# vitoplantamura/OnnxStream

Hardware: NVIDIA H100
Metric: SD1.5 UNet 512x512 bs=1 denoise steps/s (one UNet Model::run per step) (higher is better)
Workload: dtype f16

## Files before the change

### onnxstream_b200/csrc/attention_wgmma.cu

```cuda

#include "common.cuh"
#include "tc_ptx.cuh"
#include <cuda.h>
#include <cstdio>

namespace {

using namespace tcptx;

constexpr int BQ = 128;
constexpr int BKV = 128;
constexpr int KV_STAGES = 4;
constexpr int FA_THREADS = 384;
constexpr int FA_CONSUMERS = 256;
constexpr int FA_PRODUCER_REGS = 40, FA_CONSUMER_REGS = 232;

template <int NCH, int BK, int QKS, int KS = KV_STAGES, int PLANES = 1>
struct FaCfg {
    static_assert(QKS <= 4 * NCH && (BK == 32 || BK == 64 || BK == 128), "tile");
    static constexpr int Q_CHUNK = BQ * 128;
    static constexpr int KV_CHUNK = BK * 128;
    static constexpr int Q_PLANE = NCH * Q_CHUNK;
    static constexpr int KV_PLANE = NCH * KV_CHUNK;
    static constexpr int Q_BYTES = PLANES * Q_PLANE;
    static constexpr int KV_BYTES = PLANES * KV_PLANE;
    static constexpr int BARS = Q_BYTES + KS * 2 * KV_BYTES;
    static constexpr int SMEM = BARS + 1024 + 256;
};

struct FaParams {
    int T, Tk, d;
    int kv_tiles;
    float scale_log2;
    __half* out;
    long long ldo;
};

__device__ __forceinline__ uint8_t* fa_prologue(const CUtensorMap* map_q, const CUtensorMap* map_k, const CUtensorMap* map_v, int bar_off,
                                                uint32_t arrivals, int n0, int n1 = 0)
{
    extern __shared__ uint8_t smem_raw[];
    uint8_t* smem = (uint8_t*)(((uintptr_t)smem_raw + 1023) & ~(uintptr_t)1023);
    const int warp = threadIdx.x >> 5, lane = threadIdx.x & 31;
    if (warp == 0 && lane == 0) {
        asm volatile("prefetch.tensormap [%0];" ::"l"(map_q) : "memory");
        asm volatile("prefetch.tensormap [%0];" ::"l"(map_k) : "memory");
        asm volatile("prefetch.tensormap [%0];" ::"l"(map_v) : "memory");
    }
    if (warp == 1 && lane == 0) {
        uint64_t* bars = (uint64_t*)(smem + bar_off);
        mbar_init(bars, 1);
        for (int i = 0; i < n0; i++) { mbar_init(&bars[1 + i], 1); mbar_init(&bars[1 + n0 + i], arrivals); }
        for (int i = 0; i < n1; i++) { mbar_init(&bars[1 + 2 * n0 + i], 1); mbar_init(&bars[1 + 2 * n0 + n1 + i], arrivals); }
        asm volatile("fence.mbarrier_init.release.cluster;" ::: "memory");
    }
    __syncthreads();
    osb_pdl_wait();
    return smem;
}

template <int KS, typename Load>
__device__ __forceinline__ void fa_produce_kv(uint64_t* kv_full, uint64_t* kv_empty, int n_kv, uint32_t tile_bytes, Load load)
{
    for (int j = 0; j < n_kv; j++) {
        const int st = j % KS;
        mbar_wait(&kv_empty[st], ((j / KS) & 1) ^ 1);
        if (elect_one()) {
            mbar_expect_tx(&kv_full[st], tile_bytes);
            load(st, j, &kv_full[st]);
        }
        __syncwarp();
    }
    osb_pdl_trigger_late();
}

template <int BK>
__device__ __forceinline__ float fa_row_max(const float (&s)[BK / 2], int h)
{
    float mt = -INFINITY;
#pragma unroll
    for (int c = 0; c < BK / 8; c++) mt = fmaxf(mt, fmaxf(s[4 * c + 2 * h], s[4 * c + 2 * h + 1]));
    mt = fmaxf(mt, __shfl_xor_sync(0xffffffffu, mt, 1));
    mt = fmaxf(mt, __shfl_xor_sync(0xffffffffu, mt, 2));
    return mt;
}

__device__ __forceinline__ float ex2_approx(float x)
{
    float y;
    asm("ex2.approx.ftz.f32 %0, %1;" : "=f"(y) : "f"(x));
    return y;
}

__device__ __forceinline__ uint32_t pack_half2(float lo, float hi)
{
    __half2 h2 = __floats2half2_rn(lo, hi);
    return *reinterpret_cast<uint32_t*>(&h2);
}

__device__ __forceinline__ void store_pair(__half* p, float lo, float hi) { *reinterpret_cast<uint32_t*>(p) = pack_half2(lo, hi); }
__device__ __forceinline__ void store_pair(float* p, float lo, float hi) { *reinterpret_cast<float2*>(p) = make_float2(lo, hi); }

template <typename OutT, int NCH>
__device__ __forceinline__ void fa_store(const float (&o)[NCH][32], const float (&l_run)[2], OutT* const (&rows)[2], int ncols, int cq)
{
#pragma unroll
    for (int h = 0; h < 2; h++) {
        float l = l_run[h];
        l += __shfl_xor_sync(0xffffffffu, l, 1);
        l += __shfl_xor_sync(0xffffffffu, l, 2);
        const float inv = 1.f / l;
        if (!rows[h]) continue;
#pragma unroll
        for (int ch = 0; ch < NCH; ch++)
#pragma unroll
            for (int c = 0; c < 8; c++) {
                const int col = 64 * ch + 8 * c + cq;
                if (col < ncols) store_pair(rows[h] + col, o[ch][4 * c + 2 * h] * inv, o[ch][4 * c + 2 * h + 1] * inv);
            }
    }
}

template <int BK>
__device__ __forceinline__ void qk_mma(float (&s)[BK / 2], uint64_t da, uint64_t db, uint32_t scale_d = 1u)
{
    if constexpr (BK == 128) wgmma_m64n128k16_f16<0>(s, da, db, scale_d);
    else if constexpr (BK == 64) wgmma_m64n64k16_f16<0>(s, da, db, scale_d);
    else wgmma_m64n32k16_f16<0>(s, da, db, scale_d);
}

template <int NCH, int BK, int QKS>
__device__ __forceinline__ void fa_issue_qk(float (&s)[BK / 2], uint64_t qdesc, uint64_t kdesc)
{
    using C = FaCfg<NCH, BK, QKS>;
    fence_regs(s);
    wgmma_fence();
#pragma unroll
    for (int k = 0; k < QKS; k++)
        qk_mma<BK>(s, qdesc + (uint64_t)(((k >> 2) * C::Q_CHUNK >> 4) + (k & 3) * 2), kdesc + (uint64_t)(((k >> 2) * C::KV_CHUNK >> 4) + (k & 3) * 2), k > 0);
    wgmma_commit();
}

template <int NCH, int BK, int QKS>
__device__ __forceinline__ void fa_issue_pv(float (&o)[NCH][32], uint32_t (&a)[BK / 16][4], uint64_t vdesc)
{
    using C = FaCfg<NCH, BK, QKS>;
#pragma unroll
    for (int ch = 0; ch < NCH; ch++) fence_regs(o[ch]);
    fence_regs(a);
    wgmma_fence();
#pragma unroll
    for (int kk = 0; kk < BK / 16; kk++)
#pragma unroll
        for (int ch = 0; ch < NCH; ch++)
            wgmma_m64n64k16_f16_rs(o[ch], a[kk], vdesc + (uint64_t)((ch * C::KV_CHUNK + kk * 2048) >> 4), 1u);
    wgmma_commit();
}

template <int BK>
__device__ __forceinline__ void fa_softmax(float (&s)[BK / 2], float (&m_run)[2], float (&l_run)[2], float (&alpha)[2], int key0, int cq, const FaParams& p)
{
    if (key0 + BK > p.Tk) {
#pragma unroll
        for (int c = 0; c < BK / 8; c++)
#pragma unroll
            for (int e = 0; e < 2; e++)
                if (key0 + 8 * c + cq + e >= p.Tk) { s[4 * c + e] = -INFINITY; s[4 * c + 2 + e] = -INFINITY; }
    }
    float neg_m[2];
#pragma unroll
    for (int h = 0; h < 2; h++) {
        const float m_new = fmaxf(m_run[h], fa_row_max<BK>(s, h) * p.scale_log2);
        alpha[h] = ex2_approx(m_run[h] - m_new);
        neg_m[h] = -m_new;
        m_run[h] = m_new;
    }
    float lsum[2] = { 0.f, 0.f };
#pragma unroll
    for (int c = 0; c < BK / 8; c++)
#pragma unroll
        for (int h = 0; h < 2; h++)
#pragma unroll
            for (int e = 0; e < 2; e++) {
                const float pe = ex2_approx(fmaf(s[4 * c + 2 * h + e], p.scale_log2, neg_m[h]));
                s[4 * c + 2 * h + e] = pe;
                lsum[h] += pe;
            }
#pragma unroll
    for (int h = 0; h < 2; h++) l_run[h] = l_run[h] * alpha[h] + lsum[h];
}

template <int NCH, int BK>
__device__ __forceinline__ void fa_rescale_pack(float (&o)[NCH][32], uint32_t (&a)[BK / 16][4], const float (&s)[BK / 2], const float (&alpha)[2])
{
#pragma unroll
    for (int ch = 0; ch < NCH; ch++)
#pragma unroll
        for (int c = 0; c < 8; c++)
#pragma unroll
            for (int h = 0; h < 2; h++) { o[ch][4 * c + 2 * h] *= alpha[h]; o[ch][4 * c + 2 * h + 1] *= alpha[h]; }
#pragma unroll
    for (int c = 0; c < BK / 8; c++)
#pragma unroll
        for (int h = 0; h < 2; h++) a[c >> 1][(c & 1) * 2 + h] = pack_half2(s[4 * c + 2 * h], s[4 * c + 2 * h + 1]);
}

template <int NCH, int BK, int QKS>
__global__ void __launch_bounds__(FA_THREADS, 1)
flash_attention_kernel(const __grid_constant__ CUtensorMap map_q, const __grid_constant__ CUtensorMap map_k, const __grid_constant__ CUtensorMap map_v,
                       const FaParams p)
{
    using C = FaCfg<NCH, BK, QKS>;
    constexpr int S = KV_STAGES;
    osb_pdl_trigger_entry();
    const int warp = threadIdx.x >> 5, lane = threadIdx.x & 31;
    const int head = blockIdx.y;
    const int q0 = blockIdx.x * BQ;
    const int n_kv = p.kv_tiles;
    uint8_t* smem = fa_prologue(&map_q, &map_k, &map_v, C::BARS, FA_CONSUMERS / 32, S);
    uint8_t* sQ = smem;
    uint8_t* sK = sQ + C::Q_BYTES;
    uint8_t* sV = sK + S * C::KV_BYTES;
    uint64_t* q_full = (uint64_t*)(smem + C::BARS);
    uint64_t* kv_full = q_full + 1;
    uint64_t* kv_empty = kv_full + S;

    if (warp < 4) {
        setmaxnreg_dec<FA_PRODUCER_REGS>();
        if (warp == 0) {
            if (elect_one()) {
                mbar_expect_tx(q_full, C::Q_BYTES);
#pragma unroll
                for (int c = 0; c < NCH; c++) tma_load_3d(sQ + c * C::Q_CHUNK, &map_q, q_full, 64 * c, head, q0);
            }
            __syncwarp();
            fa_produce_kv<S>(kv_full, kv_empty, n_kv, 2 * C::KV_BYTES, [&](int st, int j, uint64_t* bar) {
#pragma unroll
                for (int c = 0; c < NCH; c++) {
                    tma_load_3d(sK + st * C::KV_BYTES + c * C::KV_CHUNK, &map_k, bar, 64 * c, head, j * BK);
                    tma_load_3d(sV + st * C::KV_BYTES + c * C::KV_CHUNK, &map_v, bar, 64 * c, head, j * BK);
                }
            });
        }
    } else {
        setmaxnreg_inc<FA_CONSUMER_REGS>();
        const int wg = (warp >> 2) - 1;
        const int r = (warp & 3) * 16 + (lane >> 2);
        const int cq = 2 * (lane & 3);
        const uint32_t my_bar = 1 + wg, other_bar = 2 - wg;
        if (wg == 0) named_bar_arrive(my_bar, FA_CONSUMERS);
        const uint64_t qdesc = make_smem_desc(smem_u32(sQ) + wg * (BQ / 2) * 128, 16, 1024);
        const uint64_t kdesc0 = make_smem_desc(smem_u32(sK), 16, 1024);
        const uint64_t vdesc0 = make_smem_desc(smem_u32(sV), C::KV_CHUNK, 1024);
        float o[NCH][32];
#pragma unroll
        for (int ch = 0; ch < NCH; ch++)
#pragma unroll
            for (int i = 0; i < 32; i++) o[ch][i] = 0.f;
        float s[BK / 2];
        uint32_t a[BK / 16][4];
        float m_run[2] = { -INFINITY, -INFINITY }, l_run[2] = { 0.f, 0.f }, alpha[2];
        mbar_wait(q_full, 0);

        mbar_wait(&kv_full[0], 0);
        named_bar_sync(my_bar, FA_CONSUMERS);
        fa_issue_qk<NCH, BK, QKS>(s, qdesc, kdesc0);
        named_bar_arrive(other_bar, FA_CONSUMERS);
        wgmma_wait<0>();
        fence_regs(s);
        fa_softmax<BK>(s, m_run, l_run, alpha, 0, cq, p);
        fa_rescale_pack<NCH, BK>(o, a, s, alpha);
        for (int j = 1; j < n_kv; j++) {
            const int st = j % S, prev = (j - 1) % S;
            mbar_wait(&kv_full[st], (j / S) & 1);
            named_bar_sync(my_bar, FA_CONSUMERS);
            fa_issue_qk<NCH, BK, QKS>(s, qdesc, kdesc0 + (uint64_t)(st * C::KV_BYTES >> 4));
            fa_issue_pv<NCH, BK, QKS>(o, a, vdesc0 + (uint64_t)(prev * C::KV_BYTES >> 4));
            named_bar_arrive(other_bar, FA_CONSUMERS);
            wgmma_wait<1>();
            fence_regs(s);
            fa_softmax<BK>(s, m_run, l_run, alpha, j * BK, cq, p);
            wgmma_wait<0>();
#pragma unroll
            for (int ch = 0; ch < NCH; ch++) fence_regs(o[ch]);
            fence_regs(a);
            __syncwarp();
            if (lane == 0) mbar_arrive(&kv_empty[prev]);
            fa_rescale_pack<NCH, BK>(o, a, s, alpha);
        }
        named_bar_sync(my_bar, FA_CONSUMERS);
        fa_issue_pv<NCH, BK, QKS>(o, a, vdesc0 + (uint64_t)((n_kv - 1) % S * C::KV_BYTES >> 4));
        if (wg == 0) named_bar_arrive(other_bar, FA_CONSUMERS);
        wgmma_wait<0>();
#pragma unroll
        for (int ch = 0; ch < NCH; ch++) fence_regs(o[ch]);
        __half* rows[2];
#pragma unroll
        for (int h = 0; h < 2; h++) {
            const int qrow = q0 + wg * (BQ / 2) + r + 8 * h;
            rows[h] = qrow < p.T ? p.out + (long long)qrow * p.ldo + (long long)head * p.d : nullptr;
        }
        fa_store(o, l_run, rows, p.d, cq);
    }
}

template <auto Kernel, typename... Args>
int fa_launch_kernel(dim3 grid, int threads, int smem, cudaStream_t st, const Args&... args)
{
    static bool attr = false;
    if (!attr) {
        cudaError_t e = cudaFuncSetAttribute(Kernel, cudaFuncAttributeMaxDynamicSharedMemorySize, smem);
        if (e != cudaSuccess) return (int)e;
        attr = true;
    }
    osb_launch(Kernel, grid, threads, (size_t)smem, st, args...);
    return launched(1);
}

struct SdpaParams {
    int rows;
    int Tq, Tk, d;
    int kv_tiles;
    float scale_log2;
    const __half* mask;
    __half* out;
};

__device__ __forceinline__ uint32_t ld_mask_pair(const __half* row, int col, int Tk, bool vec)
{
    const unsigned short* m = reinterpret_cast<const unsigned short*>(row) + col;
    if (col + 1 < Tk) {
        if (vec) return __ldg(reinterpret_cast<const unsigned int*>(m));
        return (uint32_t)__ldg(m) | ((uint32_t)__ldg(m + 1) << 16);
    }
    return col < Tk ? (uint32_t)__ldg(m) : 0u;
}

template <int NCH, int BK>
__global__ void __launch_bounds__(FA_THREADS, 1)
sdpa_flash_kernel(const __grid_constant__ CUtensorMap map_q, const __grid_constant__ CUtensorMap map_k, const __grid_constant__ CUtensorMap map_v,
                  const SdpaParams p)
{
    using C = FaCfg<NCH, BK, 4 * NCH>;
    constexpr float LOG2E = 1.4426950408889634f;
    osb_pdl_trigger_entry();
    const int warp = threadIdx.x >> 5, lane = threadIdx.x & 31;
    const int r0 = blockIdx.x * BQ, hk = blockIdx.y;
    const int n_kv = p.kv_tiles;
    uint8_t* smem = fa_prologue(&map_q, &map_k, &map_v, C::BARS, FA_CONSUMERS, KV_STAGES);
    uint8_t* sQ = smem;
    uint8_t* sK = sQ + C::Q_BYTES;
    uint8_t* sV = sK + KV_STAGES * C::KV_BYTES;
    uint64_t* q_full = (uint64_t*)(smem + C::BARS);
    uint64_t* kv_full = q_full + 1;
    uint64_t* kv_empty = kv_full + KV_STAGES;

    if (warp == 0) {
        if (elect_one()) {
            mbar_expect_tx(q_full, C::Q_BYTES);
#pragma unroll
            for (int c = 0; c < NCH; c++) tma_load_3d(sQ + c * C::Q_CHUNK, &map_q, q_full, 64 * c, r0, hk);
        }
        __syncwarp();
        fa_produce_kv<KV_STAGES>(kv_full, kv_empty, n_kv, 2 * C::KV_BYTES, [&](int st, int j, uint64_t* bar) {
#pragma unroll
            for (int c = 0; c < NCH; c++) {
                tma_load_3d(sK + st * C::KV_BYTES + c * C::KV_CHUNK, &map_k, bar, 64 * c, j * BK, hk);
                tma_load_3d(sV + st * C::KV_BYTES + c * C::KV_CHUNK, &map_v, bar, 64 * c, j * BK, hk);
            }
        });
    } else if (warp >= 4) {
        const int wg = (warp >> 2) - 1;
        const int r = (warp & 3) * 16 + (lane >> 2);
        const int cq = 2 * (lane & 3);
        const uint64_t qdesc = make_smem_desc(smem_u32(sQ) + wg * (BQ / 2) * 128, 16, 1024);
        const uint64_t kdesc0 = make_smem_desc(smem_u32(sK), 16, 1024);
        const uint64_t vdesc0 = make_smem_desc(smem_u32(sV), C::KV_CHUNK, 1024);
        const bool has_mask = p.mask != nullptr, vec = (p.Tk & 1) == 0;
        const __half* mrow[2];
#pragma unroll
        for (int h = 0; h < 2; h++) {
            const int R = r0 + wg * (BQ / 2) + r + 8 * h;
// ... 5 lines not shown
#pragma unroll
            for (int i = 0; i < 32; i++) o[ch][i] = 0.f;
        float m_run[2] = { -INFINITY, -INFINITY }, l_run[2] = { 0.f, 0.f };
        mbar_wait(q_full, 0);
        for (int j = 0; j < n_kv; j++) {
            const int ks = j % KV_STAGES;
            const int key0 = j * BK;
            mbar_wait(&kv_full[ks], (j / KV_STAGES) & 1);
            float s[BK / 2];
            fa_issue_qk<NCH, BK, 4 * NCH>(s, qdesc, kdesc0 + (uint64_t)(ks * C::KV_BYTES >> 4));
            uint32_t mk[2][BK / 8];
#pragma unroll
            for (int h = 0; h < 2; h++)
#pragma unroll
                for (int c = 0; c < BK / 8; c++) mk[h][c] = has_mask ? ld_mask_pair(mrow[h], key0 + 8 * c + cq, p.Tk, vec) : 0u;
            wgmma_wait<0>();
            const bool tail = key0 + BK > p.Tk;
#pragma unroll
            for (int c = 0; c < BK / 8; c++)
#pragma unroll
                for (int h = 0; h < 2; h++) {
                    __half2 m2 = *reinterpret_cast<__half2*>(&mk[h][c]);
                    const float2 mf = __half22float2(m2);
                    float x0 = fmaf(s[4 * c + 2 * h], p.scale_log2, mf.x * LOG2E);
                    float x1 = fmaf(s[4 * c + 2 * h + 1], p.scale_log2, mf.y * LOG2E);
                    if (tail) {
                        if (key0 + 8 * c + cq >= p.Tk) x0 = -INFINITY;
                        if (key0 + 8 * c + cq + 1 >= p.Tk) x1 = -INFINITY;
                    }
                    s[4 * c + 2 * h] = x0; s[4 * c + 2 * h + 1] = x1;
                }
            float alpha[2], neg_m[2];
#pragma unroll
            for (int h = 0; h < 2; h++) {
                const float m_new = fmaxf(m_run[h], fa_row_max<BK>(s, h));
                const bool none = m_new == -INFINITY;
                alpha[h] = none ? 1.f : ex2_approx(m_run[h] - m_new);
                neg_m[h] = none ? 0.f : -m_new;
                m_run[h] = m_new;
            }
            float lsum[2] = { 0.f, 0.f };
#pragma unroll
            for (int c = 0; c < BK / 8; c++) {
#pragma unroll
                for (int h = 0; h < 2; h++) {
                    const float p0 = ex2_approx(s[4 * c + 2 * h] + neg_m[h]);
                    const float p1 = ex2_approx(s[4 * c + 2 * h + 1] + neg_m[h]);
                    lsum[h] += p0 + p1;
                    s[4 * c + 2 * h] = p0; s[4 * c + 2 * h + 1] = p1;
                }
            }
#pragma unroll
            for (int h = 0; h < 2; h++) l_run[h] = l_run[h] * alpha[h] + lsum[h];
            uint32_t a[BK / 16][4];
            fa_rescale_pack<NCH, BK>(o, a, s, alpha);
            fa_issue_pv<NCH, BK, 4 * NCH>(o, a, vdesc0 + (uint64_t)(ks * C::KV_BYTES >> 4));
            wgmma_wait<0>();
            mbar_arrive(&kv_empty[ks]);
        }
        __half* rows[2];
#pragma unroll
        for (int h = 0; h < 2; h++) {
            const int R = r0 + wg * (BQ / 2) + r + 8 * h;
            rows[h] = R < p.rows ? p.out + ((long long)hk * p.rows + R) * p.d : nullptr;
        }
        fa_store(o, l_run, rows, p.d, cq);
    }
}

template <int NCH, int BK>
int sdpa_launch(const void* q, const void* k, const void* v, SdpaParams p, int64_t Hkv, cudaStream_t st)
{
    using C = FaCfg<NCH, BK, 4 * NCH>;
    const uint64_t d = p.d;
    CUtensorMap mq, mk, mv;
    if (!make_map(&mq, q, d, p.rows, Hkv, d * 2, p.rows * d * 2, 64, BQ, 1) || !make_map(&mk, k, d, p.Tk, Hkv, d * 2, p.Tk * d * 2, 64, BK, 1) ||
        !make_map(&mv, v, d, p.Tk, Hkv, d * 2, p.Tk * d * 2, 64, BK, 1))
        return (int)cudaErrorInvalidValue;
    p.kv_tiles = (p.Tk + BK - 1) / BK;
    dim3 grid((unsigned)((p.rows + BQ - 1) / BQ), (unsigned)Hkv);
    return fa_launch_kernel<sdpa_flash_kernel<NCH, BK>>(grid, FA_THREADS, C::SMEM, st, mq, mk, mv, p);
}

template <int NCH, int BK, int QKS>
int fa_launch(const void* q, int64_t ldq, const void* k, int64_t ldk, const void* v, int64_t ldv, FaParams p, int64_t heads, cudaStream_t st)
{
    using C = FaCfg<NCH, BK, QKS>;
    const uint64_t d = p.d;
    CUtensorMap mq, mk, mv;
    if (!make_map(&mq, q, d, heads, p.T, d * 2, ldq * 2, 64, 1, BQ) || !make_map(&mk, k, d, heads, p.Tk, d * 2, ldk * 2, 64, 1, BK) ||
        !make_map(&mv, v, d, heads, p.Tk, d * 2, ldv * 2, 64, 1, BK))
        return (int)cudaErrorInvalidValue;
    p.kv_tiles = (p.Tk + BK - 1) / BK;
    dim3 grid((unsigned)((p.T + BQ - 1) / BQ), (unsigned)heads);
    return fa_launch_kernel<flash_attention_kernel<NCH, BK, QKS>>(grid, FA_THREADS, C::SMEM, st, mq, mk, mv, p);
}

constexpr int WD_BQ = 64;
constexpr int WD_BK = 64;
constexpr int WD_NV = 4;
constexpr int WD_DCH = 8;
constexpr int WD_K_STAGES = 8, WD_V_STAGES = 2;
constexpr int WD_THREADS = 256, WD_CONSUMERS = 128;
constexpr int WD_PRODUCER_REGS = 40, WD_CONSUMER_REGS = 240;
constexpr int WD_Q_CHUNK = WD_BQ * 128;
constexpr int WD_K_CHUNK = WD_BK * 128;
constexpr int WD_V_CHUNK = WD_BK * 128;
constexpr int WD_V_BYTES = WD_NV * WD_V_CHUNK;
constexpr int WD_BARS = WD_DCH * WD_Q_CHUNK + WD_K_STAGES * WD_K_CHUNK + WD_V_STAGES * WD_V_BYTES;
constexpr int WD_SMEM = WD_BARS + 1024 + 256;

template <bool KT>
__device__ __forceinline__ void wd_issue_qk_chunk(float (&s)[WD_BK / 2], uint64_t qdesc, uint64_t kdesc, bool first)
{
#pragma unroll
    for (int k = 0; k < 4; k++)
        wgmma_m64n64k16_f16<KT ? 1 : 0>(s, qdesc + (uint64_t)(k * 2), kdesc + (uint64_t)(KT ? (k * 2048) >> 4 : k * 2), (first && k == 0) ? 0u : 1u);
    wgmma_commit();
}

__device__ __forceinline__ void wd_issue_pv(float (&o)[WD_NV][32], uint32_t (&a)[WD_BK / 16][4], uint64_t vdesc)
{
#pragma unroll
    for (int ch = 0; ch < WD_NV; ch++) fence_regs(o[ch]);
    fence_regs(a);
    wgmma_fence();
#pragma unroll
    for (int kk = 0; kk < WD_BK / 16; kk++)
#pragma unroll
        for (int ch = 0; ch < WD_NV; ch++)
            wgmma_m64n64k16_f16_rs(o[ch], a[kk], vdesc + (uint64_t)((ch * WD_V_CHUNK + kk * 2048) >> 4), 1u);
    wgmma_commit();
}

template <bool KT>
__global__ void __launch_bounds__(WD_THREADS, 1)
flash_attention_wide_kernel(const __grid_constant__ CUtensorMap map_q, const __grid_constant__ CUtensorMap map_k,
                            const __grid_constant__ CUtensorMap map_v, const FaParams p)
{
    constexpr int KS = WD_K_STAGES, VS = WD_V_STAGES;
    osb_pdl_trigger_entry();
    const int warp = threadIdx.x >> 5, lane = threadIdx.x & 31;
    const int n_slices = (p.d + 64 * WD_NV - 1) / (64 * WD_NV);
    const int col0 = (blockIdx.x % n_slices) * (64 * WD_NV);
    const int q0 = (blockIdx.x / n_slices) * WD_BQ;
    const int head = blockIdx.y;
    const int n_dch = (p.d + 63) >> 6;
    uint8_t* smem = fa_prologue(&map_q, &map_k, &map_v, WD_BARS, WD_CONSUMERS / 32, KS, VS);
    uint8_t* sQ = smem;
    uint8_t* sK = sQ + WD_DCH * WD_Q_CHUNK;
    uint8_t* sV = sK + KS * WD_K_CHUNK;
    uint64_t* q_full = (uint64_t*)(smem + WD_BARS);
    uint64_t* k_full = q_full + 1;
    uint64_t* k_empty = k_full + KS;
    uint64_t* v_full = k_empty + KS;
    uint64_t* v_empty = v_full + VS;
    const int n_kv = p.kv_tiles;

    if (warp < 4) {
        setmaxnreg_dec<WD_PRODUCER_REGS>();
        if (warp == 0) {
            if (elect_one()) {
                mbar_expect_tx(q_full, n_dch * WD_Q_CHUNK);
                for (int c = 0; c < n_dch; c++) tma_load_3d(sQ + c * WD_Q_CHUNK, &map_q, q_full, 64 * c, q0, head);
            }
            __syncwarp();
            const int n_vch = min(WD_NV, (p.d - col0 + 63) >> 6);
            int kc = 0;
            for (int j = 0; j < n_kv; j++) {
                for (int c = 0; c < n_dch; c++, kc++) {
                    const int st = kc % KS;
                    mbar_wait(&k_empty[st], ((kc / KS) & 1) ^ 1);
                    if (elect_one()) {
                        mbar_expect_tx(&k_full[st], WD_K_CHUNK);
                        if (KT) tma_load_3d(sK + st * WD_K_CHUNK, &map_k, &k_full[st], j * WD_BK, 64 * c, head);
                        else tma_load_3d(sK + st * WD_K_CHUNK, &map_k, &k_full[st], 64 * c, j * WD_BK, head);
                    }
                    __syncwarp();
// ... 244 lines not shown
#pragma unroll
            for (int ch = 0; ch < NCH; ch++)
#pragma unroll
                for (int c = 0; c < 8; c++)
#pragma unroll
                    for (int h = 0; h < 2; h++) { o[ch][4 * c + 2 * h] *= alpha[h]; o[ch][4 * c + 2 * h + 1] *= alpha[h]; }
            uint32_t a[3][BK / 16][4];
#pragma unroll
            for (int c = 0; c < BK / 8; c++)
#pragma unroll
                for (int h = 0; h < 2; h++) {
                    __nv_bfloat16 p0[3], p1[3];
                    bf16x3_split(s[4 * c + 2 * h], p0[0], p0[1], p0[2]);
                    bf16x3_split(s[4 * c + 2 * h + 1], p1[0], p1[1], p1[2]);
#pragma unroll
                    for (int pl = 0; pl < 3; pl++) a[pl][c >> 1][(c & 1) * 2 + h] = pack_bf162(p0[pl], p1[pl]);
                }
#pragma unroll
            for (int pl = 0; pl < 3; pl++) fence_regs(a[pl]);
#pragma unroll
            for (int ch = 0; ch < NCH; ch++) {
                float t[32];
                fence_regs(t);
                wgmma_fence();
#pragma unroll
                for (int xx = 0; xx < 6; xx++)
#pragma unroll
                    for (int kk = 0; kk < BK / 16; kk++) {
                        const int x = 5 - xx;
                        wgmma_m64n64k16_bf16_rs(t, a[x3a(x)][kk], vdesc + (uint64_t)((x3b(x) * C::KV_PLANE + ch * C::KV_CHUNK + kk * 2048) >> 4), (kk | xx) != 0);
                    }
                wgmma_commit();
                wgmma_wait<0>();
                fence_regs(t);
#pragma unroll
                for (int i = 0; i < 32; i++) o[ch][i] += t[i];
            }
#pragma unroll
            for (int pl = 0; pl < 3; pl++) fence_regs(a[pl]);
            __syncwarp();
            if (lane == 0) mbar_arrive(&kv_empty[st]);
        }
        float* rows[2];
#pragma unroll
        for (int h = 0; h < 2; h++) {
            const int qrow = q0 + wg * (BQ / 2) + r + 8 * h;
            rows[h] = qrow < p.T ? out + (long long)qrow * p.ldo + (long long)head * p.d : nullptr;
        }
        fa_store(o, l_run, rows, p.d, cq);
    }
}

template <int NCH, int BK, int QKS, int KS>
int f32x_launch(const float* q, int64_t ldq, const float* k, int64_t ldk, const float* v, int64_t ldv, float* out, FaParams p, float scale,
                int64_t heads, __nv_bfloat16* planes, cudaStream_t st)
{
    using Cf = FaCfg<NCH, BK, QKS, KS, 3>;
    const int64_t C = heads * p.d;
    const uint64_t d = p.d;
    __nv_bfloat16* pq = planes;
    __nv_bfloat16* pk = pq + 3 * p.T * C;
    __nv_bfloat16* pv = pk + 3 * p.Tk * C;
    CUtensorMap mq, mk, mv;
    if (!make_map(&mq, pq, d, 3 * heads, p.T, d * 2, 3 * C * 2, 64, 1, BQ) || !make_map(&mk, pk, d, 3 * heads, p.Tk, d * 2, 3 * C * 2, 64, 1, BK) ||
        !make_map(&mv, pv, d, 3 * heads, p.Tk, d * 2, 3 * C * 2, 64, 1, BK))
        return (int)cudaErrorInvalidValue;
    osb_launch((f32x_split_kernel), grid_for((size_t)((p.T + 2 * (int64_t)p.Tk) * C / 4), 256), 256, 0, st, q, ldq, k, ldk, v, ldv, pq, pk, pv,
               (int64_t)p.T, (int64_t)p.Tk, (int)C);
    const int e = launched();
    if (e) return e;
    p.kv_tiles = (p.Tk + BK - 1) / BK;
    dim3 grid((unsigned)((p.T + BQ - 1) / BQ), (unsigned)heads);
    return fa_launch_kernel<flash_attention_f32x_kernel<NCH, BK, QKS, KS>>(grid, FA_THREADS, Cf::SMEM, st, mq, mk, mv, p, scale, out);
}

bool fa_dims_ok(int64_t T, int64_t Tk, int64_t d)
{
    return d >= 8 && d <= 160 && d % 8 == 0 && T >= 1 && Tk >= 1 && T <= (int64_t)INT32_MAX - BQ && Tk <= (int64_t)INT32_MAX - BKV;
}

bool fa_launch_ok(int64_t heads, float scale)
{
    return heads >= 1 && heads <= 65535 && scale > 0.f && scale < INFINITY;
}

bool aligned16(const void* a, const void* b, const void* c, const void* d, const void* e = nullptr)
{
    return (((uintptr_t)a | (uintptr_t)b | (uintptr_t)c | (uintptr_t)d | (uintptr_t)e) & 15) == 0;
}

constexpr int WX_BK = 32;
constexpr int WX_QK_STAGES = 3, WX_V_STAGES = 2;
constexpr int WX_Q_PLANE = WD_BQ * 128;
constexpr int WX_K_PLANE = WX_BK * 128;
constexpr int WX_QK_BYTES = 3 * WX_Q_PLANE + 3 * WX_K_PLANE;
constexpr int WX_V_CHUNK = WX_BK * 128;
constexpr int WX_V_PLANE = WD_NV * WX_V_CHUNK;
constexpr int WX_V_BYTES = 3 * WX_V_PLANE;
constexpr int WX_BARS = WX_QK_STAGES * WX_QK_BYTES + WX_V_STAGES * WX_V_BYTES;
constexpr int WX_SMEM = WX_BARS + 1024 + 256;
static_assert(WX_SMEM <= 227 * 1024, "shared memory");

template <bool KT>
__global__ void __launch_bounds__(256) f32x_split_k_kernel(const float* __restrict__ k, __nv_bfloat16* __restrict__ pk, int Tk, int d)
{
    osb_pdl_prologue();
    __shared__ float tile[32][33];
    const int key0 = blockIdx.x * 32, c0 = blockIdx.y * 32, head = blockIdx.z;
    const int tx = threadIdx.x, ty = threadIdx.y;
    const float* src = k + (int64_t)head * Tk * d;
    for (int i = ty; i < 32; i += 8) {
        const int key = key0 + (KT ? tx : i), c = c0 + (KT ? i : tx);
        if (key < Tk && c < d) tile[c - c0][key - key0] = KT ? src[(int64_t)c * Tk + key] : src[(int64_t)key * d + c];
    }
    __syncthreads();
    __nv_bfloat16* dst = pk + (int64_t)head * 3 * Tk * d;
    for (int i = ty; i < 32; i += 8) {
        const int key = key0 + i, c = c0 + tx;
        if (key < Tk && c < d) {
            __nv_bfloat16 h, m, l;
            bf16x3_split(tile[tx][i], h, m, l);
            const int64_t o = (int64_t)key * d + c;
            dst[o] = h;
            dst[(int64_t)Tk * d + o] = m;
            dst[2 * (int64_t)Tk * d + o] = l;
        }
    }
}

__global__ void __launch_bounds__(WD_THREADS, 1)
flash_attention_wide_f32x_kernel(const __grid_constant__ CUtensorMap map_q, const __grid_constant__ CUtensorMap map_k,
                                 const __grid_constant__ CUtensorMap map_v, const FaParams p, float scale, float* __restrict__ out)
{
    constexpr int QS = WX_QK_STAGES, VS = WX_V_STAGES;
    osb_pdl_trigger_entry();
    const int warp = threadIdx.x >> 5, lane = threadIdx.x & 31;
    const int n_slices = (p.d + 64 * WD_NV - 1) / (64 * WD_NV);
    const int col0 = (blockIdx.x % n_slices) * (64 * WD_NV);
    const int q0 = (blockIdx.x / n_slices) * WD_BQ;
    const int head = blockIdx.y;
    const int n_dch = (p.d + 63) >> 6;
    const int n_vch = min(WD_NV, (p.d - col0 + 63) >> 6);
    uint8_t* smem = fa_prologue(&map_q, &map_k, &map_v, WX_BARS, WD_CONSUMERS / 32, QS, VS);
    uint8_t* sQK = smem;
    uint8_t* sV = sQK + QS * WX_QK_BYTES;
    uint64_t* qk_full = (uint64_t*)(smem + WX_BARS) + 1;
    uint64_t* qk_empty = qk_full + QS;
    uint64_t* v_full = qk_empty + QS;
    uint64_t* v_empty = v_full + VS;
    const int n_kv = p.kv_tiles;

    if (warp < 4) {
        setmaxnreg_dec<WD_PRODUCER_REGS>();
        if (warp == 0) {
            int kc = 0;
            for (int j = 0; j < n_kv; j++) {
                for (int c = 0; c < n_dch; c++, kc++) {
                    const int st = kc % QS;
                    mbar_wait(&qk_empty[st], ((kc / QS) & 1) ^ 1);
                    if (elect_one()) {
                        uint8_t* s = sQK + st * WX_QK_BYTES;
                        mbar_expect_tx(&qk_full[st], WX_QK_BYTES);
                        for (int pl = 0; pl < 3; pl++) {
                            tma_load_3d(s + pl * WX_Q_PLANE, &map_q, &qk_full[st], pl * p.d + 64 * c, q0, head);
                            tma_load_3d(s + 3 * WX_Q_PLANE + pl * WX_K_PLANE, &map_k, &qk_full[st], 64 * c, j * WX_BK, 3 * head + pl);
                        }
// ... 269 lines not shown
                float t[32];
                fence_regs(t);
                wgmma_fence();
#pragma unroll
                for (int xx = 0; xx < 6; xx++)
#pragma unroll
                    for (int kk = 0; kk < BK / 16; kk++) {
                        const int x = 5 - xx;
                        wgmma_m64n64k16_bf16_rs(t, a[x3a(x)][kk], vdesc + (uint64_t)((x3b(x) * C::KV_PLANE + ch * C::KV_CHUNK + kk * 2048) >> 4), (kk | xx) != 0);
                    }
                wgmma_commit();
                wgmma_wait<0>();
                fence_regs(t);
#pragma unroll
                for (int i = 0; i < 32; i++) o[ch][i] += t[i];
            }
#pragma unroll
            for (int pl = 0; pl < 3; pl++) fence_regs(a[pl]);
            __syncwarp();
            if (lane == 0) mbar_arrive(&kv_empty[st]);
        }
        float* rows[2];
#pragma unroll
        for (int h = 0; h < 2; h++) {
            const int R = r0 + wg * (BQ / 2) + r + 8 * h;
            rows[h] = R < p.rows ? p.out + ((long long)hk * p.rows + R) * p.d : nullptr;
        }
        fa_store(o, l_run, rows, p.d, cq);
    }
}

template <int NCH, int BK, int QKS, int KS>
int sdpa_f32x_launch(const float* q, const float* k, const float* v, SdpaF32xParams p, int64_t Hkv, __nv_bfloat16* planes, cudaStream_t st)
{
    using Cf = FaCfg<NCH, BK, QKS, KS, 3>;
    const int64_t rows = p.rows, Tk = p.Tk, d = p.d;
    __nv_bfloat16* pq = planes;
    __nv_bfloat16* pk = pq + 3 * Hkv * rows * d;
    __nv_bfloat16* pv = pk + 3 * Hkv * Tk * d;
    CUtensorMap mq, mk, mv;
    if (!make_map(&mq, pq, 3 * d, rows, Hkv, 3 * d * 2, rows * 3 * d * 2, 64, BQ, 1) ||
        !make_map(&mk, pk, d, Tk, 3 * Hkv, d * 2, Tk * d * 2, 64, BK, 1) ||
        !make_map(&mv, pv, 3 * d, Tk, Hkv, 3 * d * 2, Tk * 3 * d * 2, 64, BK, 1))
        return (int)cudaErrorInvalidValue;
    osb_launch((f32x_split_kernel), grid_for((size_t)(Hkv * rows * d / 4), 256), 256, 0, st, q, d, q, d, q, d, pq, pq, pq, Hkv * rows,
               (int64_t)0, (int)d);
    int e = launched();
    if (e) return e;
    osb_launch((f32x_split_kernel), grid_for((size_t)(Hkv * Tk * d / 4), 256), 256, 0, st, v, d, v, d, v, d, pv, pv, pv, Hkv * Tk,
               (int64_t)0, (int)d);
    if ((e = launched())) return e;
    const dim3 kgrid((unsigned)((Tk + 31) / 32), (unsigned)((d + 31) / 32), (unsigned)Hkv), kblock(32, 8);
    osb_launch((f32x_split_k_kernel<false>), kgrid, kblock, 0, st, k, pk, (int)Tk, (int)d);
    if ((e = launched())) return e;
    p.kv_tiles = (int)((Tk + BK - 1) / BK);
    dim3 grid((unsigned)((rows + BQ - 1) / BQ), (unsigned)Hkv);
    return fa_launch_kernel<sdpa_flash_f32x_kernel<NCH, BK, QKS, KS>>(grid, FA_THREADS, Cf::SMEM, st, mq, mk, mv, p);
}

}

int osb_f32x_split_rows(const float* x, __nv_bfloat16* planes, int64_t rows, int64_t C, cudaStream_t st)
{
    osb_launch((f32x_split_kernel), grid_for((size_t)(rows * C / 4), 256), 256, 0, st, x, C, x, C, x, C, planes, planes, planes, rows, (int64_t)0, (int)C);
    return launched();
}

extern "C" int osb_flash_attention_ok(int64_t T, int64_t Tk, int64_t d, int dtype)
{
    return dtype == OSB_F16 && T >= 64 && fa_dims_ok(T, Tk, d) && get_encode() != nullptr;
}

extern "C" int osb_flash_attention(const void* q, int64_t ldq, const void* k, int64_t ldk, const void* v, int64_t ldv, void* out, int64_t ldo,
                                   int64_t heads, int64_t T, int64_t Tk, int64_t d, float scale, void* stream)
{
    if (heads * T == 0) return 0;
    if (!fa_dims_ok(T, Tk, d) || !fa_launch_ok(heads, scale) || (ldq % 8) || (ldk % 8) || (ldv % 8) || (ldo % 8) || !aligned16(q, k, v, out))
        return (int)cudaErrorInvalidValue;
    FaParams p{};
    p.T = (int)T; p.Tk = (int)Tk; p.d = (int)d;
    p.scale_log2 = scale * 1.4426950408889634f;
    p.out = (__half*)out; p.ldo = ldo;
    cudaStream_t st = (cudaStream_t)stream;
    if (d <= 48) return fa_launch<1, 128, 3>(q, ldq, k, ldk, v, ldv, p, heads, st);
    if (d <= 64) return fa_launch<1, 128, 4>(q, ldq, k, ldk, v, ldv, p, heads, st);
    if (d <= 80) return fa_launch<2, 64, 5>(q, ldq, k, ldk, v, ldv, p, heads, st);
    if (d <= 128) return fa_launch<2, 64, 8>(q, ldq, k, ldk, v, ldv, p, heads, st);
    return fa_launch<3, 32, 10>(q, ldq, k, ldk, v, ldv, p, heads, st);
}

extern "C" int osb_flash_attention_f32x_ok(int64_t T, int64_t Tk, int64_t d, int dtype)
{
    return dtype == OSB_F32 && fa_dims_ok(T, Tk, d) && get_encode() != nullptr;
}

extern "C" int osb_flash_attention_f32x(const void* q, int64_t ldq, const void* k, int64_t ldk, const void* v, int64_t ldv, void* out, int64_t ldo,
                                        int64_t heads, int64_t T, int64_t Tk, int64_t d, float scale, void* planes, void* stream)
{
    if (!osb_flash_attention_f32x_ok(T, Tk, d, OSB_F32) || !fa_launch_ok(heads, scale)) return (int)cudaErrorInvalidValue;
    const int64_t C = heads * d;
    if (ldq < C || ldk < C || ldv < C || ldo < C || (ldq % 4) || (ldk % 4) || (ldv % 4) || (ldo % 4) || C > INT32_MAX) return (int)cudaErrorInvalidValue;
    if (!aligned16(q, k, v, out, planes)) return (int)cudaErrorInvalidValue;
    FaParams p{};
    p.T = (int)T; p.Tk = (int)Tk; p.d = (int)d;
    p.out = nullptr; p.ldo = ldo;
    const float* fq = (const float*)q; const float* fk = (const float*)k; const float* fv = (const float*)v;
    float* fo = (float*)out;
    __nv_bfloat16* pl = (__nv_bfloat16*)planes;
    cudaStream_t st = (cudaStream_t)stream;
    if (d <= 48) return f32x_launch<1, 64, 3, 2>(fq, ldq, fk, ldk, fv, ldv, fo, p, scale, heads, pl, st);
    if (d <= 64) return f32x_launch<1, 64, 4, 2>(fq, ldq, fk, ldk, fv, ldv, fo, p, scale, heads, pl, st);
    if (d <= 80) return f32x_launch<2, 32, 5, 2>(fq, ldq, fk, ldk, fv, ldv, fo, p, scale, heads, pl, st);
    if (d <= 128) return f32x_launch<2, 32, 8, 2>(fq, ldq, fk, ldk, fv, ldv, fo, p, scale, heads, pl, st);
    return f32x_launch<3, 32, 10, 1>(fq, ldq, fk, ldk, fv, ldv, fo, p, scale, heads, pl, st);
}

extern "C" int osb_flash_attention_wide_ok(int64_t T, int64_t Tk, int64_t d, int dtype)
{
    return dtype == OSB_F16 && d > 160 && d <= 64 * WD_DCH && d % 8 == 0 && T >= 1 && Tk >= 1 && T <= (int64_t)INT32_MAX - WD_BQ &&
           Tk <= (int64_t)INT32_MAX - WD_BK && get_encode() != nullptr;
}

extern "C" int osb_flash_attention_wide(const void* q, const void* k, const void* v, void* out, int64_t heads, int64_t T, int64_t Tk, int64_t d,
                                        float scale, int k_transposed, int dtype, void* stream)
{
    if (!osb_flash_attention_wide_ok(T, Tk, d, dtype) || !fa_launch_ok(heads, scale) || (k_transposed && Tk % 8) || !aligned16(q, k, v, out))
        return (int)cudaErrorInvalidValue;
    FaParams p{};
    p.T = (int)T; p.Tk = (int)Tk; p.d = (int)d;
    p.scale_log2 = scale * 1.4426950408889634f;
    p.out = (__half*)out; p.ldo = d;
    cudaStream_t st = (cudaStream_t)stream;
    return k_transposed ? wd_launch<true>(q, k, v, p, heads, st) : wd_launch<false>(q, k, v, p, heads, st);
}

extern "C" int osb_flash_attention_wide_f32x_ok(int64_t T, int64_t Tk, int64_t d, int dtype)
{
    return dtype == OSB_F32 && d > 160 && d <= 64 * WD_DCH && d % 8 == 0 && T >= 1 && Tk >= 1 && T <= (int64_t)INT32_MAX - WD_BQ &&
           Tk <= (int64_t)INT32_MAX - WX_BK && get_encode() != nullptr;
}

extern "C" int osb_flash_attention_wide_f32x(const void* q, const void* k, const void* v, void* out, int64_t heads, int64_t T, int64_t Tk,
                                             int64_t d, float scale, int k_transposed, void* planes, void* stream)
{
    if (!osb_flash_attention_wide_f32x_ok(T, Tk, d, OSB_F32) || !fa_launch_ok(heads, scale) || !aligned16(q, k, v, out, planes))
        return (int)cudaErrorInvalidValue;
    FaParams p{};
    p.T = (int)T; p.Tk = (int)Tk; p.d = (int)d;
    p.out = nullptr; p.ldo = d;
    return wx_launch((const float*)q, (const float*)k, (const float*)v, (float*)out, p, scale, heads, k_transposed != 0, (__nv_bfloat16*)planes,
                     (cudaStream_t)stream);
}

extern "C" int osb_sdpa_flash_ok(int64_t Hq, int64_t Hkv, int64_t Tq, int64_t Tk, int64_t d, int64_t dv, int dtype)
{
    return dtype == OSB_F16 && d == dv && d >= 8 && d <= 128 && d % 8 == 0 && Hkv >= 1 && Hkv <= 65535 && Hq >= Hkv && Hq % Hkv == 0 &&
           Tq >= 1 && Tk >= 1 && (Hq / Hkv) * Tq <= (int64_t)INT32_MAX - BQ && Tk <= (int64_t)INT32_MAX - BKV && get_encode() != nullptr;
}

extern "C" int osb_sdpa_flash(const void* q, const void* k, const void* v, const void* mask, void* out,
                              int64_t Hq, int64_t Hkv, int64_t Tq, int64_t Tk, int64_t d, float scale, void* stream)
{
    if (Hq * Tq * d == 0) return 0;
    if (!osb_sdpa_flash_ok(Hq, Hkv, Tq, Tk, d, d, OSB_F16)) return (int)cudaErrorInvalidValue;
    if (!aligned16(q, k, v, out) || ((uintptr_t)mask & 3) != 0) return (int)cudaErrorInvalidValue;
    SdpaParams p{};
    p.rows = (int)((Hq / Hkv) * Tq); p.Tq = (int)Tq; p.Tk = (int)Tk; p.d = (int)d;
    p.scale_log2 = scale * 1.4426950408889634f;
    p.mask = (const __half*)mask; p.out = (__half*)out;
    cudaStream_t st = (cudaStream_t)stream;
    return d <= 64 ? sdpa_launch<1, 128>(q, k, v, p, Hkv, st) : sdpa_launch<2, 64>(q, k, v, p, Hkv, st);
// ... 28 lines not shown
```

Baseline: 197.8.

## Add small-grid and short-KV flash attention variants with self-loading consumer warps

The flash attention kernel is parameterized by warpgroup count, min blocks per SM and KV stage count. Two new paths are added. When the grid is smaller than the SM count, it launches single-warpgroup 64-row CTAs with smaller KV tiles. For short-KV (Tk<=128, d<=64) cases, like SD cross-attention, it uses a 2-CTA/SM layout with no producer warp, where a consumer lane issues the TMA loads itself. Softmax also gains tree max reduction and split sum accumulators for ILP. The aim is better SM fill and less warp-specialization overhead, at the cost of more template variants and a more delicate ring-buffer handoff.

```diff
diff --git a/onnxstream_b200/csrc/attention_wgmma.cu b/onnxstream_b200/csrc/attention_wgmma.cu
--- a/onnxstream_b200/csrc/attention_wgmma.cu
+++ b/onnxstream_b200/csrc/attention_wgmma.cu
@@ -15,10 +15,10 @@
 constexpr int FA_CONSUMERS = 256;
 constexpr int FA_PRODUCER_REGS = 40, FA_CONSUMER_REGS = 232;
 
-template <int NCH, int BK, int QKS, int KS = KV_STAGES, int PLANES = 1>
+template <int NCH, int BK, int QKS, int KS = KV_STAGES, int PLANES = 1, int ROWS = BQ>
 struct FaCfg {
     static_assert(QKS <= 4 * NCH && (BK == 32 || BK == 64 || BK == 128), "tile");
-    static constexpr int Q_CHUNK = BQ * 128;
+    static constexpr int Q_CHUNK = ROWS * 128;
     static constexpr int KV_CHUNK = BK * 128;
     static constexpr int Q_PLANE = NCH * Q_CHUNK;
     static constexpr int KV_PLANE = NCH * KV_CHUNK;
@@ -85,6 +85,22 @@
     return mt;
 }
 
+template <int K0, int N, int BK>
+__device__ __forceinline__ float fa_max_tree(const float (&s)[BK / 2], int h)
+{
+    if constexpr (N == 1) return s[4 * (K0 >> 1) + 2 * h + (K0 & 1)];
+    else return fmaxf(fa_max_tree<K0, N / 2, BK>(s, h), fa_max_tree<K0 + N / 2, N / 2, BK>(s, h));
+}
+
+template <int BK>
+__device__ __forceinline__ float fa_row_max_tree(const float (&s)[BK / 2], int h)
+{
+    float mt = fa_max_tree<0, BK / 4, BK>(s, h);
+    mt = fmaxf(mt, __shfl_xor_sync(0xffffffffu, mt, 1));
+    mt = fmaxf(mt, __shfl_xor_sync(0xffffffffu, mt, 2));
+    return mt;
+}
+
 __device__ __forceinline__ float ex2_approx(float x)
 {
     float y;
@@ -129,10 +145,10 @@
     else wgmma_m64n32k16_f16<0>(s, da, db, scale_d);
 }
 
-template <int NCH, int BK, int QKS>
+template <int NCH, int BK, int QKS, int ROWS = BQ>
 __device__ __forceinline__ void fa_issue_qk(float (&s)[BK / 2], uint64_t qdesc, uint64_t kdesc)
 {
-    using C = FaCfg<NCH, BK, QKS>;
+    using C = FaCfg<NCH, BK, QKS, KV_STAGES, 1, ROWS>;
     fence_regs(s);
     wgmma_fence();
 #pragma unroll
@@ -157,7 +173,7 @@
     wgmma_commit();
 }
 
-template <int BK>
+template <int BK, bool ILP = false>
 __device__ __forceinline__ void fa_softmax(float (&s)[BK / 2], float (&m_run)[2], float (&l_run)[2], float (&alpha)[2], int key0, int cq, const FaParams& p)
 {
     if (key0 + BK > p.Tk) {
@@ -170,12 +186,12 @@
     float neg_m[2];
 #pragma unroll
     for (int h = 0; h < 2; h++) {
-        const float m_new = fmaxf(m_run[h], fa_row_max<BK>(s, h) * p.scale_log2);
+        const float m_new = fmaxf(m_run[h], (ILP ? fa_row_max_tree<BK>(s, h) : fa_row_max<BK>(s, h)) * p.scale_log2);
         alpha[h] = ex2_approx(m_run[h] - m_new);
         neg_m[h] = -m_new;
         m_run[h] = m_new;
     }
-    float lsum[2] = { 0.f, 0.f };
+    float lsum[2][2] = { { 0.f, 0.f }, { 0.f, 0.f } };
 #pragma unroll
     for (int c = 0; c < BK / 8; c++)
 #pragma unroll
@@ -184,10 +200,11 @@
             for (int e = 0; e < 2; e++) {
                 const float pe = ex2_approx(fmaf(s[4 * c + 2 * h + e], p.scale_log2, neg_m[h]));
                 s[4 * c + 2 * h + e] = pe;
-                lsum[h] += pe;
-            }
-#pragma unroll
-    for (int h = 0; h < 2; h++) l_run[h] = l_run[h] * alpha[h] + lsum[h];
+                lsum[h][ILP ? e : 0] += pe;
+            }
+#pragma unroll
+    for (int h = 0; h < 2; h++)
+        l_run[h] = l_run[h] * alpha[h] + (ILP ? lsum[h][0] + lsum[h][1] : lsum[h][0]);
 }
 
 template <int NCH, int BK>
@@ -205,19 +222,24 @@
         for (int h = 0; h < 2; h++) a[c >> 1][(c & 1) * 2 + h] = pack_half2(s[4 * c + 2 * h], s[4 * c + 2 * h + 1]);
 }
 
-template <int NCH, int BK, int QKS>
-__global__ void __launch_bounds__(FA_THREADS, 1)
+template <int WGS, int MINB>
+constexpr bool fa_self_load() { return WGS == 2 && MINB == 2; }
+
+template <int NCH, int BK, int QKS, int WGS, int MINB, int KS>
+__global__ void __launch_bounds__(128 * WGS + (fa_self_load<WGS, MINB>() ? 0 : 32), MINB)
 flash_attention_kernel(const __grid_constant__ CUtensorMap map_q, const __grid_constant__ CUtensorMap map_k, const __grid_constant__ CUtensorMap map_v,
                        const FaParams p)
 {
-    using C = FaCfg<NCH, BK, QKS>;
-    constexpr int S = KV_STAGES;
+    constexpr int ROWS = 64 * WGS, CONSUMERS = 128 * WGS;
+    constexpr bool SELF = fa_self_load<WGS, MINB>();
+    using C = FaCfg<NCH, BK, QKS, KS, 1, ROWS>;
+    constexpr int S = KS;
     osb_pdl_trigger_entry();
     const int warp = threadIdx.x >> 5, lane = threadIdx.x & 31;
     const int head = blockIdx.y;
-    const int q0 = blockIdx.x * BQ;
+    const int q0 = blockIdx.x * ROWS;
     const int n_kv = p.kv_tiles;
-    uint8_t* smem = fa_prologue(&map_q, &map_k, &map_v, C::BARS, FA_CONSUMERS / 32, S);
+    uint8_t* smem = fa_prologue(&map_q, &map_k, &map_v, C::BARS, CONSUMERS / 32, S);
     uint8_t* sQ = smem;
     uint8_t* sK = sQ + C::Q_BYTES;
     uint8_t* sV = sK + S * C::KV_BYTES;
@@ -225,31 +247,38 @@
     uint64_t* kv_full = q_full + 1;
     uint64_t* kv_empty = kv_full + S;
 
-    if (warp < 4) {
-        setmaxnreg_dec<FA_PRODUCER_REGS>();
-        if (warp == 0) {
-            if (elect_one()) {
-                mbar_expect_tx(q_full, C::Q_BYTES);
-#pragma unroll
-                for (int c = 0; c < NCH; c++) tma_load_3d(sQ + c * C::Q_CHUNK, &map_q, q_full, 64 * c, head, q0);
-            }
-            __syncwarp();
-            fa_produce_kv<S>(kv_full, kv_empty, n_kv, 2 * C::KV_BYTES, [&](int st, int j, uint64_t* bar) {
-#pragma unroll
-                for (int c = 0; c < NCH; c++) {
-                    tma_load_3d(sK + st * C::KV_BYTES + c * C::KV_CHUNK, &map_k, bar, 64 * c, head, j * BK);
-                    tma_load_3d(sV + st * C::KV_BYTES + c * C::KV_CHUNK, &map_v, bar, 64 * c, head, j * BK);
-                }
-            });
-        }
+    auto load_kv = [&](int j) {
+        const int st = j % S;
+        mbar_expect_tx(&kv_full[st], 2 * C::KV_BYTES);
+#pragma unroll
+        for (int c = 0; c < NCH; c++) {
+            tma_load_3d(sK + st * C::KV_BYTES + c * C::KV_CHUNK, &map_k, &kv_full[st], 64 * c, head, j * BK);
+            tma_load_3d(sV + st * C::KV_BYTES + c * C::KV_CHUNK, &map_v, &kv_full[st], 64 * c, head, j * BK);
+        }
+    };
+    if (!SELF && warp == 4 * WGS) {
+        if (elect_one()) {
+            mbar_expect_tx(q_full, C::Q_BYTES);
+#pragma unroll
+            for (int c = 0; c < NCH; c++) tma_load_3d(sQ + c * C::Q_CHUNK, &map_q, q_full, 64 * c, head, q0);
+        }
+        __syncwarp();
+        fa_produce_kv<S>(kv_full, kv_empty, n_kv, 2 * C::KV_BYTES, [&](int st, int j, uint64_t* bar) {
+#pragma unroll
+            for (int c = 0; c < NCH; c++) {
+                tma_load_3d(sK + st * C::KV_BYTES + c * C::KV_CHUNK, &map_k, bar, 64 * c, head, j * BK);
+                tma_load_3d(sV + st * C::KV_BYTES + c * C::KV_CHUNK, &map_v, bar, 64 * c, head, j * BK);
+            }
+        });
     } else {
-        setmaxnreg_inc<FA_CONSUMER_REGS>();
-        const int wg = (warp >> 2) - 1;
+        const int wg = warp >> 2;
         const int r = (warp & 3) * 16 + (lane >> 2);
         const int cq = 2 * (lane & 3);
         const uint32_t my_bar = 1 + wg, other_bar = 2 - wg;
-        if (wg == 0) named_bar_arrive(my_bar, FA_CONSUMERS);
-        const uint64_t qdesc = make_smem_desc(smem_u32(sQ) + wg * (BQ / 2) * 128, 16, 1024);
+        auto take_turn = [&] { if constexpr (WGS == 2) named_bar_sync(my_bar, CONSUMERS); };
+        auto pass_turn = [&] { if constexpr (WGS == 2) named_bar_arrive(other_bar, CONSUMERS); };
+        if (WGS == 2 && wg == 0) named_bar_arrive(my_bar, CONSUMERS);
+        const uint64_t qdesc = make_smem_desc(smem_u32(sQ) + wg * 64 * 128, 16, 1024);
         const uint64_t kdesc0 = make_smem_desc(smem_u32(sK), 16, 1024);
         const uint64_t vdesc0 = make_smem_desc(smem_u32(sV), C::KV_CHUNK, 1024);
         float o[NCH][32];
@@ -260,26 +289,41 @@
         float s[BK / 2];
         uint32_t a[BK / 16][4];
         float m_run[2] = { -INFINITY, -INFINITY }, l_run[2] = { 0.f, 0.f }, alpha[2];
+        const bool loader = SELF && warp == 0 && lane == 0;
+        if (loader) {
+            mbar_expect_tx(q_full, C::Q_BYTES);
+#pragma unroll
+            for (int c = 0; c < NCH; c++) tma_load_3d(sQ + c * C::Q_CHUNK, &map_q, q_full, 64 * c, head, q0);
+            for (int j = 0; j < S - 2 && j < n_kv; j++) load_kv(j);
+        }
         mbar_wait(q_full, 0);
 
         mbar_wait(&kv_full[0], 0);
-        named_bar_sync(my_bar, FA_CONSUMERS);
-        fa_issue_qk<NCH, BK, QKS>(s, qdesc, kdesc0);
-        named_bar_arrive(other_bar, FA_CONSUMERS);
+        take_turn();
+        fa_issue_qk<NCH, BK, QKS, ROWS>(s, qdesc, kdesc0);
+        pass_turn();
         wgmma_wait<0>();
         fence_regs(s);
-        fa_softmax<BK>(s, m_run, l_run, alpha, 0, cq, p);
+        fa_softmax<BK, true>(s, m_run, l_run, alpha, 0, cq, p);
         fa_rescale_pack<NCH, BK>(o, a, s, alpha);
         for (int j = 1; j < n_kv; j++) {
             const int st = j % S, prev = (j - 1) % S;
             mbar_wait(&kv_full[st], (j / S) & 1);
-            named_bar_sync(my_bar, FA_CONSUMERS);
-            fa_issue_qk<NCH, BK, QKS>(s, qdesc, kdesc0 + (uint64_t)(st * C::KV_BYTES >> 4));
+            take_turn();
+            if (SELF && warp == 0) {
+                const int t = j + S - 3;
+                if (lane == 0 && t < n_kv) {
+                    mbar_wait(&kv_empty[t % S], ((t / S) & 1) ^ 1);
+                    load_kv(t);
+                }
+                __syncwarp();
+            }
+            fa_issue_qk<NCH, BK, QKS, ROWS>(s, qdesc, kdesc0 + (uint64_t)(st * C::KV_BYTES >> 4));
             fa_issue_pv<NCH, BK, QKS>(o, a, vdesc0 + (uint64_t)(prev * C::KV_BYTES >> 4));
-            named_bar_arrive(other_bar, FA_CONSUMERS);
+            pass_turn();
             wgmma_wait<1>();
             fence_regs(s);
-            fa_softmax<BK>(s, m_run, l_run, alpha, j * BK, cq, p);
+            fa_softmax<BK, true>(s, m_run, l_run, alpha, j * BK, cq, p);
             wgmma_wait<0>();
 #pragma unroll
             for (int ch = 0; ch < NCH; ch++) fence_regs(o[ch]);
@@ -288,16 +332,17 @@
             if (lane == 0) mbar_arrive(&kv_empty[prev]);
             fa_rescale_pack<NCH, BK>(o, a, s, alpha);
         }
-        named_bar_sync(my_bar, FA_CONSUMERS);
+        if (SELF) osb_pdl_trigger_late();
+        take_turn();
         fa_issue_pv<NCH, BK, QKS>(o, a, vdesc0 + (uint64_t)((n_kv - 1) % S * C::KV_BYTES >> 4));
-        if (wg == 0) named_bar_arrive(other_bar, FA_CONSUMERS);
+        if (wg == 0) pass_turn();
         wgmma_wait<0>();
 #pragma unroll
         for (int ch = 0; ch < NCH; ch++) fence_regs(o[ch]);
         __half* rows[2];
 #pragma unroll
         for (int h = 0; h < 2; h++) {
-            const int qrow = q0 + wg * (BQ / 2) + r + 8 * h;
+            const int qrow = q0 + wg * 64 + r + 8 * h;
             rows[h] = qrow < p.T ? p.out + (long long)qrow * p.ldo + (long long)head * p.d : nullptr;
         }
         fa_store(o, l_run, rows, p.d, cq);
@@ -469,18 +514,22 @@
     return fa_launch_kernel<sdpa_flash_kernel<NCH, BK>>(grid, FA_THREADS, C::SMEM, st, mq, mk, mv, p);
 }
 
-template <int NCH, int BK, int QKS>
+template <int NCH, int BK, int QKS, int WGS, int MINB, int KS>
 int fa_launch(const void* q, int64_t ldq, const void* k, int64_t ldk, const void* v, int64_t ldv, FaParams p, int64_t heads, cudaStream_t st)
 {
-    using C = FaCfg<NCH, BK, QKS>;
+    constexpr int ROWS = 64 * WGS;
+    using C = FaCfg<NCH, BK, QKS, KS, 1, ROWS>;
+    static_assert(MINB * (C::SMEM + 1024) <= 228 * 1024, "shared memory for MINB resident CTAs");
     const uint64_t d = p.d;
     CUtensorMap mq, mk, mv;
-    if (!make_map(&mq, q, d, heads, p.T, d * 2, ldq * 2, 64, 1, BQ) || !make_map(&mk, k, d, heads, p.Tk, d * 2, ldk * 2, 64, 1, BK) ||
+    if (!make_map(&mq, q, d, heads, p.T, d * 2, ldq * 2, 64, 1, ROWS) || !make_map(&mk, k, d, heads, p.Tk, d * 2, ldk * 2, 64, 1, BK) ||
         !make_map(&mv, v, d, heads, p.Tk, d * 2, ldv * 2, 64, 1, BK))
         return (int)cudaErrorInvalidValue;
     p.kv_tiles = (p.Tk + BK - 1) / BK;
-    dim3 grid((unsigned)((p.T + BQ - 1) / BQ), (unsigned)heads);
-    return fa_launch_kernel<flash_attention_kernel<NCH, BK, QKS>>(grid, FA_THREADS, C::SMEM, st, mq, mk, mv, p);
+    dim3 grid((unsigned)((p.T + ROWS - 1) / ROWS), (unsigned)heads);
+    static_assert(!fa_self_load<WGS, MINB>() || KS >= 4, "self-loading ring: tile j + KS - 3 is loaded in iteration j");
+    return fa_launch_kernel<flash_attention_kernel<NCH, BK, QKS, WGS, MINB, KS>>(grid, 128 * WGS + (fa_self_load<WGS, MINB>() ? 0 : 32), C::SMEM, st,
+                                                                                 mq, mk, mv, p);
 }
 
 constexpr int WD_BQ = 64;
@@ -891,6 +940,13 @@
 bool fa_launch_ok(int64_t heads, float scale)
 {
     return heads >= 1 && heads <= 65535 && scale > 0.f && scale < INFINITY;
+}
+
+int fa_num_sms()
+{
+    static int n = 0;
+    if (!n) { int dev = 0; cudaGetDevice(&dev); cudaDeviceGetAttribute(&n, cudaDevAttrMultiProcessorCount, dev); if (n <= 0) n = 132; }
+    return n;
 }
 
 bool aligned16(const void* a, const void* b, const void* c, const void* d, const void* e = nullptr)
@@ -1326,11 +1382,22 @@
     p.scale_log2 = scale * 1.4426950408889634f;
     p.out = (__half*)out; p.ldo = ldo;
     cudaStream_t st = (cudaStream_t)stream;
-    if (d <= 48) return fa_launch<1, 128, 3>(q, ldq, k, ldk, v, ldv, p, heads, st);
-    if (d <= 64) return fa_launch<1, 128, 4>(q, ldq, k, ldk, v, ldv, p, heads, st);
-    if (d <= 80) return fa_launch<2, 64, 5>(q, ldq, k, ldk, v, ldv, p, heads, st);
-    if (d <= 128) return fa_launch<2, 64, 8>(q, ldq, k, ldk, v, ldv, p, heads, st);
-    return fa_launch<3, 32, 10>(q, ldq, k, ldk, v, ldv, p, heads, st);
+    if (heads * ((T + BQ - 1) / BQ) < fa_num_sms()) {
+        if (d <= 48) return fa_launch<1, 64, 3, 1, 2, 4>(q, ldq, k, ldk, v, ldv, p, heads, st);
+        if (d <= 64) return fa_launch<1, 64, 4, 1, 2, 4>(q, ldq, k, ldk, v, ldv, p, heads, st);
+        if (d <= 80) return fa_launch<2, 32, 5, 1, 2, 4>(q, ldq, k, ldk, v, ldv, p, heads, st);
+        if (d <= 128) return fa_launch<2, 32, 8, 1, 2, 4>(q, ldq, k, ldk, v, ldv, p, heads, st);
+        return fa_launch<3, 32, 10, 1, 2, 3>(q, ldq, k, ldk, v, ldv, p, heads, st);
+    }
+    if (d <= 64 && Tk <= BKV) {
+        if (d <= 48) return fa_launch<1, 64, 3, 2, 2, 5>(q, ldq, k, ldk, v, ldv, p, heads, st);
+        return fa_launch<1, 64, 4, 2, 2, 5>(q, ldq, k, ldk, v, ldv, p, heads, st);
+    }
+    if (d <= 48) return fa_launch<1, 128, 3, 2, 1, 4>(q, ldq, k, ldk, v, ldv, p, heads, st);
+    if (d <= 64) return fa_launch<1, 128, 4, 2, 1, 4>(q, ldq, k, ldk, v, ldv, p, heads, st);
+    if (d <= 80) return fa_launch<2, 64, 5, 2, 1, 4>(q, ldq, k, ldk, v, ldv, p, heads, st);
+    if (d <= 128) return fa_launch<2, 64, 8, 2, 1, 4>(q, ldq, k, ldk, v, ldv, p, heads, st);
+    return fa_launch<3, 32, 10, 2, 1, 4>(q, ldq, k, ldk, v, ldv, p, heads, st);
 }
 
 extern "C" int osb_flash_attention_f32x_ok(int64_t T, int64_t Tk, int64_t d, int dtype)
```

After: 199.4 (median of 6 runs). No clear change (+0.8%).
